# AnarchistHoneybun/map-oxidize

Measured on AMD Instinct MI355X. Metric: word-count input GB/s end-to-end at 1 and 8 MI355X; % of HBM peak, higher is better.
Workload: dtype u8

## Files before the change

map-oxidize_amd/csrc/mox_engine.hip:

```cpp
#include <fcntl.h>
#include <sys/stat.h>
#include <unistd.h>

#include <memory>

#include "mox_host.h"
#include "mox_unicode_tables.h"

namespace mox_host {

thread_local std::string g_err;

int fail(int code, const char* fmt, ...) {
  char buf[512];
  va_list ap;
  va_start(ap, fmt);
  vsnprintf(buf, sizeof buf, fmt, ap);
  va_end(ap);
  g_err = buf;
  return code;
}


int dalloc(mox_engine* e, void** p, size_t bytes) {
// ... 190 lines not shown
  memset(e->h_ctl_init, 0, sizeof(Ctl));
  e->h_ctl_init->err_utf8 = ~0ull;
  e->h_ctl_init->halo_err = ~0ull;
  return MOX_OK;
}

constexpr size_t map_lds_bytes() { return MAP_LDS_BYTES; }
size_t reduce_lds_bytes() { return RED_LDS_BYTES; }

float ev_ms(mox_engine* e, int a, int b) {
  float ms = 0;
  if (hipEventElapsedTime(&ms, e->ev[a], e->ev[b]) != hipSuccess) return 0;
  return ms;
}

void Seq::rec(int i) const {
  if ((i == 1 || i == 2) && map_ev[0]) {
    if (timing || map_only) (void)hipEventRecord(map_ev[i - 1], s);
    return;
  }
  if (timing || (map_only && (i == 1 || i == 2))) (void)hipEventRecord(e->ev[i], s);
}
void Seq::step(const char* name) const {
  if (!sync_each) return;
  hipError_t er = hipStreamSynchronize(s);
  fprintf(stderr, "[mox] %s done: %s\n", name, hipGetErrorString(er));
}

Seq seq_of(mox_engine* e) {
  const bool full = (e->flags & MOX_F_TIMING) != 0;
  return Seq{e, e->stream, full, e->sync_each, !full && (e->flags & MOX_F_TIMING_MAP) != 0};
}

void launch_reduce_tail(mox_engine* e, const Corpus& c, const Seq& q, bool zero) {
  Work& w = e->w;
  hipStream_t s = e->stream;
  hipLaunchKernelGGL(k_hist, dim3(w.map_grid), dim3(1024), 0, s, w);
  q.step("k_hist");
  hipLaunchKernelGGL(k_scatter, dim3(w.map_grid), dim3(1024), 0, s, w);
  q.step("k_scatter");
  hipLaunchKernelGGL(k_split_count, dim3(NB), dim3(256), 0, s, w);
  q.step("k_split_count");
  hipLaunchKernelGGL(k_unit_scan, dim3(1), dim3(256), 0, s, w);
  q.step("k_unit_scan");
  hipLaunchKernelGGL(k_split_scatter, dim3(NB), dim3(1024), 0, s, w);
  q.step("k_split_scatter");
  hipLaunchKernelGGL(k_reduce_sort1, dim3(MOX_S1_WG * e->n_cu), dim3(256), 0, s, w);
  q.step("k_reduce_sort1");
  hipLaunchKernelGGL(k_reduce_sort2, dim3(8 * e->n_cu), dim3(64), 0, s, w);
  q.step("k_reduce_sort2");
  hipLaunchKernelGGL(zero ? k_reduce_z : k_reduce, dim3(NB), dim3(RED_THREADS), reduce_lds_bytes(), s, w);
  q.step("k_reduce");
  hipLaunchKernelGGL(k_reduce_small, dim3(8 * e->n_cu), dim3(128), 0, s, w);
  q.step("k_reduce_small");
  q.rec(4);
  hipLaunchKernelGGL(k_unit_uniq_scan, dim3(NB), dim3(1024), 0, s, w);
  q.step("k_unit_uniq_scan");
  hipLaunchKernelGGL(k_final_scan, dim3(1), dim3(NB), 0, s, w);
  q.step("k_final_scan");
  hipLaunchKernelGGL(k_mat, dim3(std::max(NB, 6 * e->n_cu)), dim3(256), 0, s, w, c);
  q.step("k_mat");
  q.rec(5);
}

int finish_pass(mox_engine* e, const Seq& q) {
  HIPCHK(hipGetLastError());
  HIPCHK(hipMemcpyAsync(e->h_ctl, e->w.ctl, sizeof(Ctl), hipMemcpyDeviceToHost, e->stream));
  HIPCHK(hipStreamSynchronize(e->stream));
  if (q.map_only && !q.sync_each) {
    e->stats.ms_dict = e->stats.ms_lanes = e->stats.ms_reduce = e->stats.ms_finalize = e->stats.ms_run = 0;
    e->stats.ms_map = ev_ms(e, 1, 2);
  }
  if (q.timing) {
    e->stats.ms_dict = ev_ms(e, 0, 1);
    e->stats.ms_map = ev_ms(e, 1, 2);
    e->stats.ms_lanes = ev_ms(e, 2, 3);
    e->stats.ms_reduce = ev_ms(e, 3, 4);
    e->stats.ms_finalize = ev_ms(e, 4, 5);
    e->stats.ms_run = ev_ms(e, 0, 5);
  }
  return MOX_OK;
}

void launch_dict(mox_engine* e, const Corpus& c, hipStream_t s, const Seq& q) {
  Work& w = e->w;
  hipLaunchKernelGGL(k_sample, dim3(e->sample_pieces), dim3(256), 0, s, c, w, e->sample_pieces);
  q.step("k_sample");
  hipLaunchKernelGGL(k_dict_hist, dim3(GC_SLOTS / 1024), dim3(1024), 0, s, w);
  q.step("k_dict_hist");
  hipLaunchKernelGGL(k_dict_pick, dim3(GC_SLOTS / 1024), dim3(1024), 0, s, w, e->dict_words);
  q.step("k_dict_pick");
  hipLaunchKernelGGL(k_dict_build, dim3(1), dim3(1024), 0, s, w, e->dict_words);
  q.step("k_dict_build");
}

void enqueue_pass(mox_engine* e, const Corpus& c, const Seq& q, bool side = false) {
  Work& w = e->w;
  hipStream_t s = e->stream;
  q.rec(0);
  const bool dict = !(e->flags & MOX_F_NO_DICT) && c.own_hi > c.own_lo;
  const bool sided = side && dict && !q.timing && !q.sync_each;
  if (sided) {
    use_dset(e, e->dcur ^ 1);
    if (e->mapped_pending) (void)hipStreamWaitEvent(e->dstream, e->ev_mapped, 0);
    e->mapped_pending = false;
    hipLaunchKernelGGL(k_dict_zero, dim3(64), dim3(256), 0, e->dstream, w);
    launch_dict(e, c, e->dstream, q);
    (void)hipEventRecord(e->ev_dready, e->dstream);
  }
  hipLaunchKernelGGL(k_init, dim3(256), dim3(256), 0, s, w, 0ull, sided ? 4u : (dict ? 1u : 0u));
  q.step("k_init");
  if (sided) (void)hipStreamWaitEvent(s, e->ev_dready, 0);
  else if (dict) launch_dict(e, c, s, q);
  q.rec(1);
  const uint64_t row0 = c.own_lo & ~15ull;
  const uint64_t nrows = c.own_hi > c.own_lo ? (c.own_hi - row0 + PAY - 1) / PAY : 0;
  const int grid = (int)w.map_grid;
  hipLaunchKernelGGL(k_map, dim3(grid), dim3(MAP_THREADS), map_lds_bytes(), s, c, w, nrows, 0u);
  q.step("k_map");
  q.rec(2);
#ifndef MOX_SIDE_AFTER_MAP
#define MOX_SIDE_AFTER_MAP 0
#endif
  if (MOX_SIDE_AFTER_MAP && side && !q.timing && !q.sync_each) {
    (void)hipEventRecord(e->ev_mapped, s);
    e->mapped_pending = true;
  }
  hipLaunchKernelGGL(k_unicode, dim3(1024), dim3(256), 0, s, c, w, e->tables);
  q.step("k_unicode");
  q.rec(3);
  launch_reduce_tail(e, c, q, false);
}

int pipeline_once(mox_engine* e, const Corpus& c) {
  const Seq q = seq_of(e);
  enqueue_pass(e, c, q);
  return finish_pass(e, q);
}

uint64_t cold_cap_for(const mox_engine* e, const Ctl& h) {
  const uint64_t want = h.cold_need + h.cold_need / 8 + 16;
  const uint64_t bound = 4 * h.tokens / ((uint64_t)e->w.map_grid * NB) + 64;
  return std::min(want, std::max<uint64_t>(bound, e->w.cold_cap));
}

Caps grow_for(mox_engine* e, const Ctl& h) {
  Caps need = caps_of(e->w);
  if (h.overflow & OVF_POOL) {
    need.cold_cap = std::max<uint64_t>(need.cold_cap, cold_cap_for(e, h));
    need.spill_cap = std::max<uint64_t>(need.spill_cap, h.spill_need + h.spill_need / 4 + 1024);
  }
  if (h.overflow & OVF_W) {
    const uint64_t wn = std::max<uint64_t>(h.w_total, h.w_n);
    need.w_cap = std::max<uint64_t>(need.w_cap, wn + wn / 4 + 1024);
  }
  if (h.overflow & OVF_U) need.u_cap = h.u_n + h.u_n / 4 + 1024;
  if (h.overflow & OVF_ARENA) need.arena_cap = h.arena_n + h.arena_n / 4 + 65536;
  if (h.overflow & OVF_LONG) need.long_cap = next_pow2(2 * h.long_n + 1024);
  if (h.overflow & OVF_TABLE) need.table_cap = h.n_total + h.n_total / 4 + 1024;
  if (h.overflow & OVF_BYTES) need.bytes_cap = h.bytes_total + h.bytes_total / 4 + 65536;
  if (h.overflow & OVF_SPLIT) {
    uint64_t k = h.split_k + h.split_k / 8 + 4096, wv = h.split_w + h.split_w / 8 + 4096;
    if (need.split_k_cap || need.split_w_cap) {
      k = std::max<uint64_t>(k, h.cold_recs + h.cold_recs / 8 + (uint64_t)NB * (SUB_N + 2));
      wv = std::max<uint64_t>(wv, h.w_total + h.w_total / 8 + 4096);
    }
    need.split_k_cap = std::max<uint64_t>(need.split_k_cap, k);
    need.split_w_cap = std::max<uint64_t>(need.split_w_cap, wv);
  }
  if (h.overflow & OVF_TABLE) need.bytes_cap = std::max(need.bytes_cap, need.table_cap * 16);
  return need;
}

void commit_result(mox_engine* e, const Corpus& c, const Ctl& h);

void set_result(mox_engine* e, const Ctl& h) {
  e->res.counts = e->w.t_counts;
  e->res.offs = e->w.t_offs;
  e->res.bytes = e->w.t_bytes;
  e->res.n = h.n_total;
  e->res.nb = h.bytes_total;
  e->res.tokens = h.tokens;
  e->res.pass = true;
  e->res.exchanged = false;
  e->res.sorted = false;
  e->res.ranked = false;
  e->res.folded = false;
  e->have_result = true;
}
// ... 129 lines not shown
  if (&h != e->h_ctl) std::memcpy(e->h_ctl, &h, sizeof(Ctl));
  if (h.spill_need) e->next_cold_cap = std::max<uint64_t>(e->next_cold_cap, cold_cap_for(e, h));
  e->stats.bytes = c.own_hi - c.own_lo;
  e->stats.tokens = h.tokens;
  e->stats.uniques = h.n_total;
  e->stats.dict_words = h.dict_n;
  e->stats.cold_records = h.cold_recs;
  e->stats.weighted_records = h.w_n;
  e->stats.unicode_tokens = h.u_n;
  e->stats.long_tokens = h.long_n;
  e->stats.chunks = h.cold_need;
  e->stats.max_subpasses = h.max_sub ? h.max_sub : 1;
  e->stats.reduce_units = h.n_units;
  e->stats.split_partitions = h.n_split;
  static_assert(sizeof(e->stats.path_hits) == sizeof(h.paths), "path counters");
  std::memcpy(e->stats.path_hits, h.paths, sizeof h.paths);
  e->last_corpus = c;
  set_result(e, h);
}

int complete_async(mox_engine* e, int k) {
  auto& a = e->aslot[k];
  if (!a.pending) return MOX_OK;
  a.pending = false;
  HIPCHK(hipEventSynchronize(a.ev_done));
  const Ctl& h = *a.h_ctl;
  auto& later = e->aslot[k ^ 1];
  if (int rc = check_failed(h)) return rc;
  if (h.err_utf8 != ~0ull) return fail(MOX_EUTF8, "stream did not contain valid UTF-8 (byte %llu)", h.err_utf8);
  if (h.halo_err != ~0ull)
    return fail(MOX_EHALO, "token at byte %llu runs past the end of a non-final shard buffer", h.halo_err);
  if (!h.overflow) {
    const bool map_only = (e->flags & (MOX_F_TIMING | MOX_F_TIMING_MAP)) != 0;
    if (map_only) {
      float ms = 0;
      if (hipEventElapsedTime(&ms, a.ev_map0, a.ev_map1) == hipSuccess) e->stats.ms_map = ms;
    }
    e->stats.retries = 0;
    commit_result(e, a.c, h);
    if (later.pending) e->have_result = false;
    return MOX_OK;
  }
  if (later.pending) {
    e->grow_hint = caps_max(e->grow_hint, grow_for(e, h));
    e->stats.async_dropped++;
    return MOX_OK;
  }
  HIPCHK(hipStreamSynchronize(e->stream));
  if (e->dstream) HIPCHK(hipStreamSynchronize(e->dstream));
  e->stats.async_reruns++;
  return run_corpus(e, a.c);
}

int drain_async(mox_engine* e) {
  const int first = e->anext;
  int rc = complete_async(e, first);
  const int rc2 = complete_async(e, first ^ 1);
  if (e->dstream) HIPCHK(hipStreamSynchronize(e->dstream));
  return rc ? rc : rc2;
}

Corpus make_corpus(const void* d_buf, size_t buf_len, size_t own_begin, size_t own_end, int at_end) {
  uintptr_t addr = (uintptr_t)d_buf;
  uint64_t mis = (addr & 15) + 16;
  Corpus c{};
  c.base = (const uint8_t*)(addr - mis);
  c.lo = mis;
  c.hi = mis + buf_len;
  c.own_lo = mis + own_begin;
  c.own_hi = mis + own_end;
  c.ctx_lo = mis;
  c.at_end = at_end ? 1 : 0;
  return c;
}


int engine_create_one(const mox_config* cfg, int dev, mox_engine** out) {
  *out = nullptr;
  mox_engine* e = new (std::nothrow) mox_engine();
  if (!e) return fail(MOX_ENOMEM, "host allocation failed");
  if (cfg) {
    e->flags = cfg->flags;
    if (cfg->dict_words) e->dict_words = std::min<uint32_t>(cfg->dict_words, DICT_MAX_WORDS);
    if (cfg->sample_pieces) e->sample_pieces = std::min<uint32_t>(cfg->sample_pieces, MAX_SAMPLE_PIECES);
  }
  int ndev = 0;
  if (hipGetDeviceCount(&ndev) != hipSuccess || ndev == 0) {
    delete e;
    return fail(MOX_EHIP, "no HIP device available");
  }
  if (dev < 0) {
    if (hipGetDevice(&dev) != hipSuccess) dev = 0;
  }
  if (dev >= ndev) {
    delete e;
    return fail(MOX_EINVAL, "device %d out of range (%d devices)", dev, ndev);
  }
  e->device = dev;
  hipError_t herr = hipSetDevice(dev);
  if (herr != hipSuccess) { delete e; return fail(MOX_EHIP, "hipSetDevice: %s", hipGetErrorString(herr)); }
  hipDeviceProp_t prop;
  if (hipGetDeviceProperties(&prop, dev) == hipSuccess) e->n_cu = prop.multiProcessorCount;
  if (hipStreamCreateWithFlags(&e->stream, hipStreamNonBlocking) != hipSuccess) {
    delete e;
    return fail(MOX_EHIP, "hipStreamCreate failed");
  }
  for (auto& ev : e->ev) (void)hipEventCreate(&ev);
  if (hipStreamCreateWithFlags(&e->dstream, hipStreamNonBlocking) != hipSuccess ||
      hipEventCreateWithFlags(&e->ev_dready, hipEventDisableTiming) != hipSuccess ||
      hipEventCreateWithFlags(&e->ev_mapped, hipEventDisableTiming) != hipSuccess) {
    mox_engine_destroy(e);
    return fail(MOX_EHIP, "side stream / events: creation failed");
  }
  if (hipFuncSetAttribute((const void*)k_map, hipFuncAttributeMaxDynamicSharedMemorySize, (int)map_lds_bytes()) != hipSuccess ||
      hipFuncSetAttribute((const void*)k_reduce, hipFuncAttributeMaxDynamicSharedMemorySize, (int)reduce_lds_bytes()) != hipSuccess ||
      hipFuncSetAttribute((const void*)k_reduce_z, hipFuncAttributeMaxDynamicSharedMemorySize, (int)reduce_lds_bytes()) != hipSuccess) {
    mox_engine_destroy(e);
    return fail(MOX_EHIP, "hipFuncSetAttribute(dynamic LDS) failed");
  }
  if (const char* d = getenv("MOX_DBG")) e->w.dbg = (uint32_t)strtoul(d, nullptr, 0);
  if (e->w.dbg & DBG_STAMP) (void)hipMalloc((void**)&e->w.stamps, 8 * 8 * 4096 + 8 * 8 * 1024 * MAP_WAVES + 8 * 4 * 1024 * 16);
  e->sync_each = getenv("MOX_SYNC_EACH") != nullptr;
  e->verbose = getenv("MOX_VERBOSE") != nullptr;
  if (const char* f = getenv("MOX_TEST_FAIL_ALLOC")) e->test_fail_alloc = atoi(f);
  int rc = alloc_fixed(e);
  if (rc == MOX_OK && cfg && cfg->reserve_bytes) rc = ensure_caps(e, initial_caps(cfg->reserve_bytes, e->n_cu));
  if (rc != MOX_OK) {
    std::string msg = g_err;
    mox_engine_destroy(e);
    g_err = msg;
    return rc;
  }
  *out = e;
  return MOX_OK;
}

int stage_host_range(mox_engine* e, const uint8_t* text, size_t len) {
  if (len > e->d_text_cap) {
    dfree(e->d_text);
    e->d_text = nullptr;
    e->d_text_cap = 0;
    int rc = dalloc(e, (void**)&e->d_text, len + 64);
    if (rc) return rc;
    e->d_text_cap = len;
  }
  const bool timing = (e->flags & MOX_F_TIMING) != 0;
  if (timing) HIPCHK(hipEventRecord(e->ev[8], e->stream));
  if (len) HIPCHK(hipMemcpyAsync(e->d_text, text, len, hipMemcpyHostToDevice, e->stream));
  if (timing) HIPCHK(hipEventRecord(e->ev[9], e->stream));
  HIPCHK(hipStreamSynchronize(e->stream));
  if (timing) e->stats.ms_h2d = ev_ms(e, 8, 9);
  return MOX_OK;
}


constexpr int MAX_FILE_READERS = 16;
int file_readers() {
  static const int n = [] {
    const char* v = getenv("MOX_FILE_READERS");
    const int k = v ? atoi(v) : 8;
    return k < 1 ? 1 : (k > MAX_FILE_READERS ? MAX_FILE_READERS : k);
  }();
  return n;
}
bool file_shared_stream() {
  static const bool one = [] {
    const char* v = getenv("MOX_FILE_STREAMS");
// ... 626 lines not shown
```

map-oxidize_amd/csrc/mox_host.h:

```cpp
#pragma once
#include <fcntl.h>
#include <sys/mman.h>
#include <sys/stat.h>
#include <unistd.h>

#include <algorithm>
#include <atomic>
#include <condition_variable>
#include <chrono>
#include <cstdarg>
#include <cstdio>
#include <cstdlib>
#include <cstring>
#include <initializer_list>
#include <mutex>
#include <string>
#include <thread>
#include <vector>

#include <rccl/rccl.h>

#include "../../include/mox.h"
#include "mox_internal.h"
#include "mox_table.h"
// ... 10 lines not shown
__global__ void k_dict_build(Work w, uint32_t max_words);
__global__ void k_dict_zero(Work w);
__global__ void k_unicode(Corpus c, Work w, Tables T);
__global__ void k_hist(Work w);
__global__ void k_scatter(Work w);
__global__ void k_reduce(Work w);
__global__ void k_reduce_z(Work w);
__global__ void k_split_count(Work w);
__global__ void k_unit_scan(Work w);
__global__ void k_split_scatter(Work w);
__global__ void k_unit_uniq_scan(Work w);
__global__ void k_final_scan(Work w);
__global__ void k_reduce_small(Work w);
__global__ void k_reduce_sort1(Work w);
__global__ void k_reduce_sort2(Work w);
__global__ void k_mat(Work w, Corpus c);
__global__ void k_xcount(Work w, uint32_t P, XCnt* xcnt);
__global__ void k_xpack_short(Work w, WRec* out);
__global__ void k_xpack_long(Work w, XDir dir, unsigned long long* cur, uint8_t* blob);
__global__ void k_xsample(Work w, uint64_t* out);
__global__ void k_xsplit(const uint64_t* blocks, uint32_t P, uint64_t* sp, uint32_t* flag);
__global__ void k_xcount_r(Work w, XSplit x, XCnt* xcnt);
__global__ void k_xpack_r(Work w, XSplit x, XDir dir, unsigned long long* cur, WRec* out, uint8_t* blob);
__global__ void k_xingest(Work w, XDir dir, uint64_t n_short);
__global__ void k_gather_offs(const uint8_t* recv, GDir d, uint64_t* out);
}

namespace mox_host {
constexpr int GROW_RETRIES = 8;


extern thread_local std::string g_err;
int fail(int code, const char* fmt, ...) __attribute__((format(printf, 2, 3)));

#define HIPCHK(expr)                                                                             \
  do {                                                                                           \
    hipError_t e_ = (expr);                                                                      \
    if (e_ != hipSuccess) return fail(MOX_EHIP, "%s failed: %s (%s:%d)", #expr, hipGetErrorString(e_), __FILE__, __LINE__); \
  } while (0)

#define RCCLCHK(expr)                                                                            \
  do {                                                                                           \
    ncclResult_t r_ = (expr);                                                                    \
    if (r_ != ncclSuccess) return fail(MOX_ERCCL, "%s failed: %s", #expr, ncclGetErrorString(r_)); \
  } while (0)

inline uint64_t next_pow2(uint64_t x) {
  uint64_t p = 1;
  while (p < x) p <<= 1;
  return p;
}

struct DevBuf {
  void* p = nullptr;
  size_t cap = 0;
};
struct Caps {
  uint64_t cold_cap, spill_cap, w_cap, u_cap, arena_cap, long_cap, table_cap, bytes_cap, split_k_cap, split_w_cap;
};
struct XPlan;
struct Group;

}

using namespace mox_host;

struct mox_engine {
  int device = 0;
  hipStream_t stream = nullptr;
  hipStream_t dstream = nullptr;
  hipEvent_t ev_dready = nullptr;
  hipEvent_t ev_mapped = nullptr;
  bool mapped_pending = false;
  struct DictSet {
    WRec* cand = nullptr;
    uint32_t* dict_hist = nullptr;
    WRec* dict_list = nullptr;
    uint32_t* dict_tag = nullptr;
    uint4* dict_key = nullptr;
    unsigned long long* dict_tot = nullptr;
  } dsets[2];
  int dcur = 0;
  uint32_t flags = 0, dict_words = DICT_MAX_WORDS, sample_pieces = 192;
  int n_cu = 256;
  bool sync_each = false;
  bool verbose = false;
  int test_fail_alloc = 0;
  uint64_t next_cold_cap = 0;
  Caps grow_hint{};
  Work w{};
  Tables tables{};
  Ctl* h_ctl = nullptr;
  Ctl* h_ctl_init = nullptr;
  uint64_t* h_tot = nullptr;
  uint8_t* d_text = nullptr;
  size_t d_text_cap = 0;
  hipStream_t file_stream[16]{};
  hipEvent_t file_ev[16][2]{};
  hipEvent_t file_land = nullptr;
  uint8_t* file_pin[16][2]{};
  size_t file_pin_bytes = 0;
  bool have_result = false;
  struct Res {
    const uint64_t* counts = nullptr;
    const uint64_t* offs = nullptr;
    const uint8_t* bytes = nullptr;
    uint64_t n = 0, nb = 0, tokens = 0;
    bool pass = false;
    bool exchanged = false;
    bool sorted = false;
    bool ranked = false;
    bool folded = false;
  } res;
  struct Acc {
    bool have = false, sorted = false, ranked = false;
    uint64_t n = 0, nb = 0, tokens = 0, passes = 0;
  } acc;
  DevBuf a_tab[3], a_tc;
  DevBuf g_counts, g_offs, g_bytes, g_recv;
  DevBuf s_counts, s_offs, s_bytes, s_tmp;
  unsigned long long* h_bsort = nullptr;
  DevBuf k_tmp, k_out;
  DevBuf tx_pre, tx_slice[2], tx_pin[2];
  hipEvent_t tx_ev[2]{};
  DevBuf l_tmp, l_pin;
  DevBuf f_tab[2][3], f_tmp;
  DevBuf r_tab[2][3], r_tmp;
  uint64_t* h_rmax = nullptr;
  DevBuf q_tc;
  Corpus last_corpus{};
  mox_stats stats{};
  hipEvent_t ev[12]{};
  struct AsyncSlot {
    bool pending = false;
    Corpus c{};
    Ctl* h_ctl = nullptr;
    hipEvent_t ev_map0 = nullptr, ev_map1 = nullptr, ev_done = nullptr;
  } aslot[2];
  int anext = 0;
  ncclComm_t comm = nullptr;
  int nranks = 1, rank = 0;
  XCnt* d_xcnt = nullptr;
  XCnt* h_xcnt = nullptr;
  unsigned long long* d_xcur = nullptr;
  uint64_t* d_xs = nullptr;
  uint64_t* d_xr = nullptr;
  uint64_t* d_xsp = nullptr;
  uint32_t* h_xflag = nullptr;
  hipEvent_t ev_xs = nullptr;
  DevBuf x_send_short, x_send_blob, x_recv_short, x_recv_blob;
  DevBuf hx_send, hx_recv;
  Ctl* h_ctl_x = nullptr;
  XPlan* xp = nullptr;
  Group* grp = nullptr;
};

namespace mox_host {
int dalloc(mox_engine* e, void** p, size_t bytes);
void dfree(void* p);
Caps caps_of(const Work& w);
Caps initial_caps(uint64_t n, int map_grid);
Caps caps_max(const Caps& a, const Caps& b);
int ensure_caps(mox_engine* e, const Caps& need);
Caps grow_for(mox_engine* e, const Ctl& h);
int check_failed(const Ctl& h);
void set_result(mox_engine* e, const Ctl& h);
// ... 61 lines not shown
```

map-oxidize_amd/csrc/mox_internal.h:

```cpp
#pragma once
#include <hip/hip_runtime.h>
#include <stdint.h>

namespace mox {

constexpr int MAP_THREADS = 1024;
constexpr int MAP_WG_PER_CU = 1;
constexpr int MAP_MIN_WAVES = 1;
#if defined(MOX_ABLATE) && !defined(MOX_EXPERIMENT_BUILD)
#error "MOX_ABLATE is an experiment build (tools/build_variant.sh): not for the product library"
#endif
constexpr int MAP_LOADERS = 1;
#ifndef MOX_LD_SLEEP
#define MOX_LD_SLEEP 1
#endif
#ifndef MOX_CO_SLEEP
#define MOX_CO_SLEEP 1
#endif
#ifndef MOX_RING
#define MOX_RING 32
#endif
constexpr int RING = MOX_RING;
#ifndef MOX_DICT_SLOTS
#define MOX_DICT_SLOTS 5120
#endif
constexpr int DICT_SLOTS = MOX_DICT_SLOTS;
constexpr int DICT_MAX_WORDS = DICT_SLOTS < 4096 ? DICT_SLOTS : 4096;
constexpr size_t DICT_CNT_BYTES = (size_t)DICT_SLOTS * 4;
static_assert(DICT_SLOTS % 32 == 0 && DICT_SLOTS <= 65536 && DICT_MAX_WORDS <= DICT_SLOTS, "dictionary geometry");
constexpr int MAX_MAP_GRID = 1024;
constexpr int MAP_WAVES = MAP_THREADS / 64;
constexpr int ROW = 1024;
constexpr int ROWBUF = ROW + 32;
constexpr int TOKMAX = ROW / 2;
constexpr int SLOT = ROW;
constexpr int PAY = ROW - 32;
constexpr int KSEL_N = 17 * 4;
#ifndef MOX_LD_GROUPS
#define MOX_LD_GROUPS 4
#endif
#ifndef MOX_LD_GROUP
#define MOX_LD_GROUP 6
#endif
constexpr int LD_GROUP = MOX_LD_GROUP;
constexpr int LD_GROUPS = MOX_LD_GROUPS;
constexpr int MAP_CONSUMERS = MAP_WAVES - MAP_LOADERS;
constexpr int MAP_ROW_WAVES = MAP_CONSUMERS;
static_assert(TOKMAX - 1 >= PAY / 2, "list[TOKMAX - 1] is the token-loop sink: no row may reach it");
constexpr int LIST_N = TOKMAX + 64;
constexpr int NB_LOG2 = 10;
constexpr int NB = 1 << NB_LOG2;
constexpr uint64_t COLD_CAP_MAX = (1ull << 32) / (16ull * NB);
constexpr uint32_t QF_MAX = 4;
constexpr size_t MAP_LDS_BYTES = (size_t)DICT_SLOTS * 16 + DICT_CNT_BYTES + NB * 4 + 16 + KSEL_N * 16 +
                                 (size_t)RING * 8 + (size_t)RING * SLOT + (size_t)MAP_ROW_WAVES * 2 * LIST_N;
static_assert(MAP_LDS_BYTES <= 160 * 1024, "k_map LDS over 160 KiB");
constexpr int GC_SLOTS = 65536;
constexpr int MAX_SAMPLE_PIECES = 1024;
constexpr int SAMPLE_PIECE = 4096;
constexpr int SAMPLE_SLOTS = 2048;
constexpr int DH_N = 258, DH_T = 259;
constexpr int RED_THREADS = 1024;
constexpr int RED_BK = 608;
constexpr int RED_BUCKETS = RED_BK + 1;
constexpr int RED_SLOTS = 4 * RED_BUCKETS;
constexpr int RED_CAP = 2048;
constexpr int RED_SORTB = 2048;
constexpr size_t RED_LDS_BYTES = (size_t)RED_SLOTS * (4 + 16 + 8) + RED_CAP * 2 + (RED_SORTB + 8) * 2 + RED_SORTB * 2 + 16;
static_assert(RED_SLOTS * 4 % 16 == 0 && RED_LDS_BYTES + 256 <= 80 * 1024, "k_reduce LDS: 2 workgroups per CU");
constexpr int SUB_BITS_MAX = 12;
constexpr int SUB_N = 1 << SUB_BITS_MAX;
constexpr int U_MAX = NB * SUB_N;
constexpr int SUB_PER_T = SUB_N / 1024;
#ifndef MOX_SPLIT_MIN
#define MOX_SPLIT_MIN 8192
#endif
constexpr uint32_t SPLIT_MIN = MOX_SPLIT_MIN;
constexpr uint32_t SPLIT_TARGET = 320;
constexpr uint32_t SMALL_CAP = 512;
#ifndef MOX_S1_WG
#define MOX_S1_WG 4
#endif
#ifndef MOX_SPLIT_PER_REGION
#define MOX_SPLIT_PER_REGION 4
#endif
constexpr uint32_t SPLIT_PER_REGION = MOX_SPLIT_PER_REGION;
constexpr uint32_t SPLIT_SAMPLE = 256 * SPLIT_PER_REGION;
constexpr int LC_BITS = 4096;

constexpr uint64_t LONG_TAG = 0xFF00000000000000ull;
constexpr uint64_t LONG_LEN_MASK = 0x0000FFFFFFFFFFFFull;
constexpr uint64_t ARENA_BIT = 1ull << 63;

#ifdef MOX_ABLATE
#define MOX_ABL(d, f) (((d) & (f)) != 0)
#else
#define MOX_ABL(d, f) (false)
#endif
enum : uint32_t { DBG_NO_TOKENS = 1u, DBG_NO_EMIT = 2u, DBG_NO_DICT = 4u, DBG_NO_COLDSTORE = 8u, DBG_NO_DICTADD = 16u,
                  DBG_RED_NOSORT = 32u, DBG_RED_NOINSERT = 64u, DBG_RED_NOSLOW = 128u, DBG_COUNT = 256u, DBG_RED_PLAINADD = 512u, DBG_STAMP = 1024u,
                  DBG_RED_TWICE = 2048u,
                  DBG_NO_ROW = 4096u,
                  DBG_PAIR_NOSTORE = 8192u,
                  DBG_NOPAIR = 16384u,
                  DBG_PAIR_SEQ = 32768u,
                  DBG_S1_SORT2 = 65536u };
enum : uint32_t {
  CHK_SMALL_DESC = 1u, CHK_SMALL_OUT = 2u, CHK_RED_OUT = 3u, CHK_SPLIT_K = 4u, CHK_SPLIT_W = 5u, CHK_UNIT = 6u,
  CHK_MAT_ROW = 7u, CHK_MAT_BYTES = 8u, CHK_SCATTER = 9u, CHK_RED_IN = 10u, CHK_GATHER = 11u,
  CHK_RED_TABLE = 12u,
  CHK_RED_NU = 13u
};
#ifdef MOX_CHECK
#define MOX_CHK(w, ok, site) (::mox::chk_record((w).ctl, (ok), (site)))
#else
#define MOX_CHK(w, ok, site) (true)
#endif
enum : uint32_t {
  OVF_POOL = 1u, OVF_W = 2u, OVF_U = 4u, OVF_LONG = 8u, OVF_ARENA = 16u, OVF_PROBE = 32u,
  OVF_TABLE = 64u, OVF_BYTES = 128u, OVF_REDUCE = 256u, OVF_SPLIT = 512u,
  OVF_RERUN = OVF_POOL | OVF_W | OVF_U | OVF_LONG | OVF_ARENA | OVF_PROBE | OVF_SPLIT
};

struct Ctl {
  unsigned long long w_n;
  unsigned long long u_n;
  unsigned long long arena_n;
  unsigned long long long_n;
  unsigned long long long_uniq;
  unsigned long long tokens;
  unsigned long long err_utf8;
  unsigned long long halo_err;
  unsigned long long cold_recs;
  unsigned long long n_short;
  unsigned long long n_total;
  unsigned long long bytes_total;
  unsigned int overflow;
  unsigned int dict_n;
  unsigned int dict_maxprobe;
  unsigned int max_sub;
  unsigned int dict_thresh;
  unsigned int done[3];
  unsigned long long cold_need;
// ... 236 lines not shown
```

map-oxidize_amd/csrc/mox_kernels.hip:

```cpp
#include "mox_internal.h"

namespace mox {

__device__ __forceinline__ uint32_t movemask8(uint64_t m80) {
  uint64_t m = (m80 >> 7) & 0x0101010101010101ull;
  m |= m >> 7;
  m |= m >> 14;
  m |= m >> 28;
  return (uint32_t)m & 0xFFu;
}
__device__ __forceinline__ uint64_t zero_bytes80(uint64_t v) {
  uint64_t t = (v & 0x7F7F7F7F7F7F7F7Full) + 0x7F7F7F7F7F7F7F7Full;
  return ~(t | v | 0x7F7F7F7F7F7F7F7Full);
}
__device__ __forceinline__ uint64_t ws_bytes80(uint64_t x) {
  uint64_t sp = zero_bytes80(x ^ 0x2020202020202020ull);
  uint64_t ge9 = x + 0x7777777777777777ull;
  uint64_t ge14 = x + 0x7272727272727272ull;
  return (sp | (ge9 & ~ge14)) & 0x8080808080808080ull;
}
__device__ __forceinline__ uint64_t lower_ascii(uint64_t x) {
  uint64_t ge_a = x + 0x3F3F3F3F3F3F3F3Full;
  uint64_t gt_z = x + 0x2525252525252525ull;
  return x | (((ge_a & ~gt_z) & 0x8080808080808080ull) >> 2);
// ... 991 lines not shown
    for (uint32_t j = cnt; j < SPLIT_PER_REGION; j++) note_sample(m, b, q, j, 0u);
    cmax = cnt > cmax ? cnt : cmax;
  }
  for (int off = 32; off > 0; off >>= 1) {
    ntok += __shfl_down(ntok, off);
    const uint32_t o = __shfl_down(cmax, off);
    cmax = o > cmax ? o : cmax;
  }
  if (lane == 0) {
    if (ntok) atomicAdd(&s_tok, ntok);
    if (cmax) atomicMax(&s_cmax, cmax);
  }
  __syncthreads();
  if (tid == 0) {
    const uint32_t sn = m.s.misc[0];
    w.spill_n[blockIdx.x] = sn < w.spill_cap ? sn : w.spill_cap;
    if (sn) atomicMax(&w.ctl->spill_need, sn);
    if (s_cmax) atomicMax(&w.ctl->cold_need, (unsigned long long)s_cmax * m.qf);
    if (s_tok) atomicAdd(&w.ctl->tokens, s_tok);
    if (blockIdx.x == 0) w.ctl->qf = m.qf;
  }
}

extern "C" __global__ void k_ctl_out(const Ctl* __restrict__ src, Ctl* __restrict__ dst) {
  constexpr int CW = sizeof(Ctl) / 8;
  const int t = threadIdx.x;
  if (t < CW) reinterpret_cast<volatile unsigned long long*>(dst)[t] = reinterpret_cast<const unsigned long long*>(src)[t];
}

enum : uint32_t { INIT_DICT = 1u, INIT_MAP = 2u, INIT_DICT_SIDE = 4u };
__device__ __forceinline__ void zero_words(void* p, uint64_t bytes, uint64_t t, uint64_t stride) {
  uint4* q = reinterpret_cast<uint4*>(p);
  const uint64_t n16 = bytes / 16;
  for (uint64_t i = t; i < n16; i += stride) q[i] = make_uint4(0, 0, 0, 0);
  uint32_t* r = reinterpret_cast<uint32_t*>(q + n16);
  for (uint64_t i = t; i < (bytes % 16) / 4; i += stride) r[i] = 0;
}
extern "C" __global__ void k_init(Work w, unsigned long long w_n, uint32_t flags) {
  const uint64_t t = (uint64_t)blockIdx.x * blockDim.x + threadIdx.x, stride = (uint64_t)gridDim.x * blockDim.x;
  constexpr int CW = sizeof(Ctl) / 8;
  static_assert(sizeof(Ctl) % 8 == 0, "Ctl is zeroed in 8-byte words");
  if (t < CW) {
    unsigned long long* c = reinterpret_cast<unsigned long long*>(w.ctl);
    const uint64_t off = t * 8;
    unsigned long long v = 0;
    if (off == offsetof(Ctl, err_utf8) || off == offsetof(Ctl, halo_err)) v = ~0ull;
    if (off == offsetof(Ctl, w_n)) v = w_n;
    c[t] = v;
  }
  zero_words(w.b_recs, NB * 8, t, stride);
  zero_words(w.b_w, NB * 4, t, stride);
  zero_words(w.ltab, w.long_cap * sizeof(LSlot), t, stride);
  if (flags & INIT_DICT) {
    zero_words(w.cand, (uint64_t)GC_SLOTS * sizeof(WRec), t, stride);
    zero_words(w.dict_hist, 260 * 4, t, stride);
  }
  if (flags & (INIT_DICT | INIT_DICT_SIDE)) zero_words(w.dict_tot, DICT_SLOTS * 8, t, stride);
  else if (t == 0) { w.dict_hist[DH_N] = 0; w.dict_hist[DH_T] = 0; }
  if (flags & INIT_MAP) {
    zero_words(w.cold_n, (uint64_t)w.map_grid * NB * QF_MAX * 4, t, stride);
    zero_words(w.samp, (uint64_t)w.map_grid * NB * QF_MAX * SPLIT_PER_REGION * 4, t, stride);
    zero_words(w.spill_n, (uint64_t)w.map_grid * 4, t, stride);
  }
}

extern "C" __global__ void k_dict_zero(Work w) {
  const uint64_t t = (uint64_t)blockIdx.x * blockDim.x + threadIdx.x, stride = (uint64_t)gridDim.x * blockDim.x;
  zero_words(w.cand, (uint64_t)GC_SLOTS * sizeof(WRec), t, stride);
  zero_words(w.dict_hist, 260 * 4, t, stride);
}
__device__ __forceinline__ bool claim16(unsigned long long* k0, unsigned long long* k1, uint64_t w0, uint64_t w1) {
  const unsigned long long t1 = w1 | (1ull << 63);
  unsigned long long o0 = atomicCAS(k0, 0ull, (unsigned long long)w0);
  if (o0 != 0 && o0 != w0) return false;
  unsigned long long o1 = atomicCAS(k1, 0ull, t1);
  return o1 == 0 || o1 == t1;
}

__device__ __forceinline__ uint32_t lower32(uint32_t x) {
  const uint32_t ge_a = x + 0x3F3F3F3Fu, gt_z = x + 0x25252525u;
  return x | (((ge_a & ~gt_z) & 0x80808080u) >> 2);
}

extern "C" __global__ __launch_bounds__(256) void k_sample(Corpus c, Work w, uint32_t npieces) {
  constexpr int BUF = SAMPLE_PIECE + 48;
  __shared__ __attribute__((aligned(16))) uint8_t buf[BUF];
  __shared__ unsigned long long sk0[SAMPLE_SLOTS], sk1[SAMPLE_SLOTS];
  __shared__ uint32_t scnt[SAMPLE_SLOTS];
  __shared__ uint4 mtab[17];
  const int tid = threadIdx.x;
  for (int i = tid; i < SAMPLE_SLOTS; i += 256) { sk0[i] = 0; sk1[i] = 0; scnt[i] = 0; }
  if (tid < 17) {
    uint32_t mk[4];
#pragma unroll
    for (int i = 0; i < 4; i++) {
      const int cc = tid - 4 * i;
      mk[i] = cc <= 0 ? 0u : (cc >= 4 ? ~0u : ((1u << (8 * cc)) - 1u));
    }
    mtab[tid] = make_uint4(mk[0], mk[1], mk[2], mk[3]);
  }
  const uint64_t span = c.own_hi - c.own_lo;
  const uint64_t stride = span / npieces;
  const uint64_t ps = (c.own_lo + stride * blockIdx.x) & ~15ull;
  for (int i = tid; i < BUF / 16; i += 256) {
    const uint64_t p = ps - 16 + (uint64_t)i * 16;
    const bool in = p + 16 > c.lo && p < c.hi;
    reinterpret_cast<uint4*>(buf)[i] = in ? fix16(c, p, raw16(c, p)) : make_uint4(0x20202020u, 0x20202020u, 0x20202020u, 0x20202020u);
  }
  __syncthreads();
  const uint4 own = reinterpret_cast<const uint4*>(buf)[1 + tid], nxt = reinterpret_cast<const uint4*>(buf)[2 + tid];
  const uint32_t prevb = buf[15 + 16 * tid];
  const uint32_t ws32 = ws_mask16(own) | (ws_mask16(nxt) << 16);
  uint32_t start = (~ws32) & ((ws32 << 1) | (is_ascii_ws(prevb) ? 1u : 0u)) & 0xFFFFu;
  while (start) {
    const uint32_t p = __builtin_ctz(start);
    start &= start - 1;
    const uint32_t rest = ws32 >> p;
    const uint32_t len = rest ? __builtin_ctz(rest) : 32;
    if (len > 16) continue;
    const uint32_t pos = 16 + 16 * tid + p;
    const uint2* q = reinterpret_cast<const uint2*>(buf + (pos & ~7u));
    const uint2 A = q[0], B = q[1], C = q[2];
    const uint4 M = mtab[len];
    const bool o = (pos & 4u) != 0;
    const uint32_t E0 = o ? A.y : A.x, E1 = o ? B.x : A.y, E2 = o ? B.y : B.x, E3 = o ? C.x : B.y, E4 = o ? C.y : C.x;
    const uint32_t sh = pos & 3u;
    uint32_t K[4] = {__builtin_amdgcn_alignbyte(E1, E0, sh) & M.x, __builtin_amdgcn_alignbyte(E2, E1, sh) & M.y,
                     __builtin_amdgcn_alignbyte(E3, E2, sh) & M.z, __builtin_amdgcn_alignbyte(E4, E3, sh) & M.w};
    if (((K[0] | K[1] | K[2] | K[3]) & 0x80808080u) != 0) continue;
    const uint32_t nz = (uint32_t)__popcll(zero_bytes80(((uint64_t)K[1] << 32) | K[0])) +
                        (uint32_t)__popcll(zero_bytes80(((uint64_t)K[3] << 32) | K[2]));
    if (nz != 16 - len) continue;
#pragma unroll
    for (int i = 0; i < 4; i++) K[i] = lower32(K[i]);
    const uint64_t w0 = ((uint64_t)K[1] << 32) | K[0], w1 = ((uint64_t)K[3] << 32) | K[2];
    uint32_t slot = hash32(K[0], K[1], K[2], K[3]) & (SAMPLE_SLOTS - 1);
    for (int pr = 0; pr < 64; pr++) {
      if (claim16(&sk0[slot], &sk1[slot], w0, w1)) { atomicAdd(&scnt[slot], 1u); break; }
      slot = (slot + 1) & (SAMPLE_SLOTS - 1);
    }
  }
  __syncthreads();
  __shared__ uint16_t lw[SAMPLE_SLOTS];
  __shared__ uint32_t nlw;
  if (tid == 0) nlw = 0;
  __syncthreads();
  for (int i = tid; i < SAMPLE_SLOTS; i += 256) {
    const bool used = scnt[i] != 0 && sk0[i] != 0 && sk1[i] != 0;
    const uint64_t bm = __ballot(used);
    uint32_t b0 = 0;
    if ((tid & 63) == 0 && bm) b0 = atomicAdd(&nlw, (uint32_t)__popcll(bm));
    b0 = __shfl(b0, 0);
    if (used) lw[b0 + (uint32_t)__popcll(bm & ((1ull << (tid & 63)) - 1ull))] = (uint16_t)i;
  }
  __syncthreads();
  for (uint32_t j = tid; j < nlw; j += 256) {
    const uint32_t i = lw[j];
    const uint32_t n = scnt[i];
    const uint64_t w0 = sk0[i], w1 = sk1[i] & ~(1ull << 63);
    uint32_t g = key_hash(w0, w1) & (GC_SLOTS - 1);
    for (int pr = 0; pr < 16; pr++) {
      WRec* r = &w.cand[g];
      if (claim16((unsigned long long*)&r->w0, (unsigned long long*)&r->w1, w0, w1)) {
        atomicAdd((unsigned long long*)&r->count, (unsigned long long)n);
        break;
      }
      g = (g + 1) & (GC_SLOTS - 1);
    }
  }
}

extern "C" __global__ __launch_bounds__(1024) void k_dict_hist(Work w) {
  __shared__ uint32_t h[256];
  if (threadIdx.x < 256) h[threadIdx.x] = 0;
  __syncthreads();
  for (uint32_t i = blockIdx.x * 1024 + threadIdx.x; i < GC_SLOTS; i += gridDim.x * 1024) {
    const uint64_t n = w.cand[i].count;
    if (n) atomicAdd(&h[n > 255 ? 255 : n], 1u);
  }
  __syncthreads();
  if (threadIdx.x < 256 && h[threadIdx.x]) atomicAdd(&w.dict_hist[threadIdx.x], h[threadIdx.x]);
}

constexpr uint32_t DICT_MIN_COVER_INV = 20;
extern "C" __global__ __launch_bounds__(1024) void k_dict_pick(Work w, uint32_t max_words) {
  __shared__ uint32_t T, ST, h[256];
  __shared__ unsigned long long cov[2];
  if (threadIdx.x < 256) h[threadIdx.x] = w.dict_hist[threadIdx.x];
  __syncthreads();
  {
    __shared__ uint64_t wsum[16];
    uint64_t tot;
    const int cc = 255 - (int)threadIdx.x;
    const uint64_t x = threadIdx.x < 256 ? h[cc] : 0;
    const uint64_t ex = block_exscan(x, wsum, tot);
    if (threadIdx.x == 0) { T = 256; ST = 0; }
    __syncthreads();
    if (threadIdx.x < 254 && ex + x <= max_words) atomicMin(&T, (uint32_t)cc);
    __syncthreads();
    if (threadIdx.x < 256 && cc == (int)T) ST = (uint32_t)(ex + x);
    if (threadIdx.x == 0) {
      if (T > 255) T = 256;
      cov[0] = 0;
      cov[1] = 0;
    }
    __syncthreads();
    if (threadIdx.x < 256 && cc >= 1 && x) {
      const unsigned long long tok = x * (unsigned long long)cc;
      atomicAdd(&cov[0], tok);
      if ((uint32_t)cc >= T) atomicAdd(&cov[1], tok);
    }
    __syncthreads();
    if (threadIdx.x == 0) {
      if (cov[1] < cov[0] / DICT_MIN_COVER_INV) T = 256;
      if (blockIdx.x == 0) w.dict_hist[DH_T] = T;
    }
    __syncthreads();
  }
  __shared__ uint32_t wn[2][16], base[2];
  const uint32_t t = T, t1 = T - 1;
  const uint32_t i = blockIdx.x * 1024 + threadIdx.x;
  const WRec r = w.cand[i];
  const bool real = r.w0 != 0 && r.w1 != 0;
  const bool pick = real && r.count >= t;
  const bool fill = real && t1 >= 2 && t1 < 255 && r.count == t1;
  const uint64_t bm = __ballot(pick), bf = __ballot(fill);
  const int lane = threadIdx.x & 63, wv = threadIdx.x >> 6;
  if (lane == 0) { wn[0][wv] = (uint32_t)__popcll(bm); wn[1][wv] = (uint32_t)__popcll(bf); }
  __syncthreads();
  const uint64_t lt = (1ull << lane) - 1ull;
  uint32_t pre = (uint32_t)__popcll(bm & lt), pref = (uint32_t)__popcll(bf & lt), tot = 0, totf = 0;
  for (int k = 0; k < 16; k++) {
    if (k < wv) { pre += wn[0][k]; pref += wn[1][k]; }
    tot += wn[0][k];
    totf += wn[1][k];
  }
  if (threadIdx.x == 0) {
    base[0] = tot ? atomicAdd(&w.dict_hist[256], tot) : 0u;
    base[1] = totf ? atomicAdd(&w.dict_hist[257], totf) : 0u;
  }
  __syncthreads();
  if (pick) {
    const uint32_t o = base[0] + pre;
    if (o < max_words) w.dict_list[o] = WRec{r.w0, r.w1 & ~(1ull << 63), r.count};
  } else if (fill) {
    const uint32_t o = ST + base[1] + pref;
    if (o < max_words) w.dict_list[o] = WRec{r.w0, r.w1 & ~(1ull << 63), r.count};
  }
}

extern "C" __global__ __launch_bounds__(1024) void k_dict_build(Work w, uint32_t max_words) {
  __shared__ uint32_t ltag[DICT_SLOTS];
  __shared__ uint16_t lword[DICT_SLOTS];
  __shared__ uint32_t klock[DICT_SLOTS / 32];
  __shared__ uint2 lk0[DICT_MAX_WORDS], lk1[DICT_MAX_WORDS];
  __shared__ uint8_t lcl[DICT_MAX_WORDS];
  __shared__ uint16_t order[DICT_MAX_WORDS];
  __shared__ uint16_t fails[DICT_MAX_WORDS];
  __shared__ uint32_t ccnt[32], cstart[33], cfill[32];
  __shared__ uint32_t nsel, nfail;
  const int tid = threadIdx.x;
  for (int i = tid; i < DICT_SLOTS; i += 1024) ltag[i] = 0;
  for (int i = tid; i < DICT_SLOTS / 32; i += 1024) klock[i] = 0;
  if (tid < 32) { ccnt[tid] = 0; cfill[tid] = 0; }
  if (tid == 0) nsel = 0;
  uint32_t n = w.dict_hist[256] + w.dict_hist[257];
  if (n > max_words) n = max_words;
  __syncthreads();
  for (uint32_t i = tid; i < n; i += 1024) {
    const WRec r = w.dict_list[i];
    const uint32_t cnt = r.count > 0xFFFFFFFFull ? 0xFFFFFFFFu : (uint32_t)r.count;
    lk0[i] = make_uint2((uint32_t)r.w0, (uint32_t)(r.w0 >> 32));
    lk1[i] = make_uint2((uint32_t)r.w1, (uint32_t)(r.w1 >> 32));
    lcl[i] = (uint8_t)(31 - __clz(cnt | 1u));
    atomicAdd(&ccnt[lcl[i]], 1u);
  }
  __syncthreads();
  if (tid == 0) {
    uint32_t a = 0;
    for (int cl = 31; cl >= 0; cl--) { cstart[cl] = a; a += ccnt[cl]; }
    cstart[32] = a;
  }
  __syncthreads();
  for (uint32_t i = tid; i < n; i += 1024) order[cstart[lcl[i]] + atomicAdd(&cfill[lcl[i]], 1u)] = (uint16_t)i;
  __syncthreads();
  for (int cl = 31; cl >= 0; cl--) {
    const uint32_t c0 = cstart[cl], c1 = c0 + ccnt[cl];
    if (c0 == c1) continue;
    if (tid == 0) nfail = 0;
    __syncthreads();
    for (uint32_t j = c0 + tid; j < c1; j += 1024) {
      const uint32_t i = order[j];
      const uint2 a = lk0[i], b = lk1[i];
      const uint32_t h = hash32(a.x, a.y, b.x, b.y);
      int slot = -1;
      if (atomicCAS(&ltag[dict_s1(h)], 0u, h) == 0u) slot = (int)dict_s1(h);
      else if (atomicCAS(&ltag[dict_s2(h)], 0u, h) == 0u) slot = (int)dict_s2(h);
      if (slot < 0) { fails[atomicAdd(&nfail, 1u)] = (uint16_t)i; continue; }
      lword[slot] = (uint16_t)i;
    }
    __syncthreads();
    const uint32_t nf = nfail;
    for (uint32_t j = tid; j < nf; j += 1024) {
      const uint32_t i = fails[j];
      const uint2 a = lk0[i], b = lk1[i];
      const uint32_t h = hash32(a.x, a.y, b.x, b.y);
      const uint32_t xs[2] = {dict_s1(h), dict_s2(h)};
      for (int q = 0; q < 2; q++) {
        const uint32_t x = xs[q];
        if (atomicOr(&klock[x >> 5], 1u << (x & 31)) & (1u << (x & 31))) continue;
        const uint32_t ho = ltag[x];
        const uint32_t alt = dict_s1(ho) == x ? dict_s2(ho) : dict_s1(ho);
        if (alt == x) continue;
        if (atomicOr(&klock[alt >> 5], 1u << (alt & 31)) & (1u << (alt & 31))) continue;
// ... 1913 lines not shown
```

Baseline: 993.9.

## Shrink k_sample LDS so it co-resides with k_map and scale sample count

Rewrites k_sample to keep a small 32-bit hash-tag table in LDS (about 4 KiB) instead of a 4 KiB text buffer plus full 16-byte keys. Tokens are re-derived from registers and emitted in a second pass by their first occurrence, with overflow words going straight to the global candidate table. This lets sample workgroups fit beside the persistent k_map on the side stream. It also grows the sample count with input size up to a larger default and doubles GC_SLOTS. The cost is hash-tag collisions merging distinct words into one count, more global atomics on overflow, and more sampling work.

```diff
diff --git a/map-oxidize_amd/csrc/mox_engine.hip b/map-oxidize_amd/csrc/mox_engine.hip
--- a/map-oxidize_amd/csrc/mox_engine.hip
+++ b/map-oxidize_amd/csrc/mox_engine.hip
@@ -296,9 +296,16 @@
   return MOX_OK;
 }
 
+uint32_t sample_count(const mox_engine* e, const Corpus& c, bool side) {
+  if (!side) return e->sample_pieces;
+  const uint64_t fit = (c.own_hi - c.own_lo) / (SAMPLE_PIECE + 16);
+  return (uint32_t)std::min<uint64_t>(e->sample_pieces_max, std::max<uint64_t>(e->sample_pieces, fit));
+}
+
 void launch_dict(mox_engine* e, const Corpus& c, hipStream_t s, const Seq& q) {
   Work& w = e->w;
-  hipLaunchKernelGGL(k_sample, dim3(e->sample_pieces), dim3(256), 0, s, c, w, e->sample_pieces);
+  const uint32_t pieces = sample_count(e, c, s == e->dstream);
+  hipLaunchKernelGGL(k_sample, dim3(pieces), dim3(256), 0, s, c, w, pieces);
   q.step("k_sample");
   hipLaunchKernelGGL(k_dict_hist, dim3(GC_SLOTS / 1024), dim3(1024), 0, s, w);
   q.step("k_dict_hist");
@@ -318,7 +325,7 @@
     use_dset(e, e->dcur ^ 1);
     if (e->mapped_pending) (void)hipStreamWaitEvent(e->dstream, e->ev_mapped, 0);
     e->mapped_pending = false;
-    hipLaunchKernelGGL(k_dict_zero, dim3(64), dim3(256), 0, e->dstream, w);
+    hipLaunchKernelGGL(k_dict_zero, dim3(128), dim3(256), 0, e->dstream, w);
     launch_dict(e, c, e->dstream, q);
     (void)hipEventRecord(e->ev_dready, e->dstream);
   }
@@ -614,7 +621,7 @@
   if (cfg) {
     e->flags = cfg->flags;
     if (cfg->dict_words) e->dict_words = std::min<uint32_t>(cfg->dict_words, DICT_MAX_WORDS);
-    if (cfg->sample_pieces) e->sample_pieces = std::min<uint32_t>(cfg->sample_pieces, MAX_SAMPLE_PIECES);
+    if (cfg->sample_pieces) e->sample_pieces = e->sample_pieces_max = std::min<uint32_t>(cfg->sample_pieces, MAX_SAMPLE_PIECES);
   }
   int ndev = 0;
   if (hipGetDeviceCount(&ndev) != hipSuccess || ndev == 0) {
diff --git a/map-oxidize_amd/csrc/mox_host.h b/map-oxidize_amd/csrc/mox_host.h
--- a/map-oxidize_amd/csrc/mox_host.h
+++ b/map-oxidize_amd/csrc/mox_host.h
@@ -116,6 +116,7 @@
   } dsets[2];
   int dcur = 0;
   uint32_t flags = 0, dict_words = DICT_MAX_WORDS, sample_pieces = 192;
+  uint32_t sample_pieces_max = DEFAULT_SAMPLE_PIECES;
   int n_cu = 256;
   bool sync_each = false;
   bool verbose = false;
diff --git a/map-oxidize_amd/csrc/mox_internal.h b/map-oxidize_amd/csrc/mox_internal.h
--- a/map-oxidize_amd/csrc/mox_internal.h
+++ b/map-oxidize_amd/csrc/mox_internal.h
@@ -55,10 +55,13 @@
 constexpr size_t MAP_LDS_BYTES = (size_t)DICT_SLOTS * 16 + DICT_CNT_BYTES + NB * 4 + 16 + KSEL_N * 16 +
                                  (size_t)RING * 8 + (size_t)RING * SLOT + (size_t)MAP_ROW_WAVES * 2 * LIST_N;
 static_assert(MAP_LDS_BYTES <= 160 * 1024, "k_map LDS over 160 KiB");
-constexpr int GC_SLOTS = 65536;
-constexpr int MAX_SAMPLE_PIECES = 1024;
+constexpr int GC_SLOTS = 131072;
+constexpr int MAX_SAMPLE_PIECES = 2048;
+constexpr int DEFAULT_SAMPLE_PIECES = 768;
 constexpr int SAMPLE_PIECE = 4096;
-constexpr int SAMPLE_SLOTS = 2048;
+constexpr int SAMPLE_SLOTS = 512;
+constexpr int SAMPLE_PROBES = 8;
+static_assert(MAP_LDS_BYTES + 1280 + 4096 <= 160 * 1024, "no room for a k_sample workgroup beside k_map (1,280 B LDS granule)");
 constexpr int DH_N = 258, DH_T = 259;
 constexpr int RED_THREADS = 1024;
 constexpr int RED_BK = 608;
diff --git a/map-oxidize_amd/csrc/mox_kernels.hip b/map-oxidize_amd/csrc/mox_kernels.hip
--- a/map-oxidize_amd/csrc/mox_kernels.hip
+++ b/map-oxidize_amd/csrc/mox_kernels.hip
@@ -1097,34 +1097,33 @@
   return x | (((ge_a & ~gt_z) & 0x80808080u) >> 2);
 }
 
-extern "C" __global__ __launch_bounds__(256) void k_sample(Corpus c, Work w, uint32_t npieces) {
-  constexpr int BUF = SAMPLE_PIECE + 48;
-  __shared__ __attribute__((aligned(16))) uint8_t buf[BUF];
-  __shared__ unsigned long long sk0[SAMPLE_SLOTS], sk1[SAMPLE_SLOTS];
-  __shared__ uint32_t scnt[SAMPLE_SLOTS];
-  __shared__ uint4 mtab[17];
-  const int tid = threadIdx.x;
-  for (int i = tid; i < SAMPLE_SLOTS; i += 256) { sk0[i] = 0; sk1[i] = 0; scnt[i] = 0; }
-  if (tid < 17) {
-    uint32_t mk[4];
-#pragma unroll
-    for (int i = 0; i < 4; i++) {
-      const int cc = tid - 4 * i;
-      mk[i] = cc <= 0 ? 0u : (cc >= 4 ? ~0u : ((1u << (8 * cc)) - 1u));
-    }
-    mtab[tid] = make_uint4(mk[0], mk[1], mk[2], mk[3]);
-  }
-  const uint64_t span = c.own_hi - c.own_lo;
-  const uint64_t stride = span / npieces;
-  const uint64_t ps = (c.own_lo + stride * blockIdx.x) & ~15ull;
-  for (int i = tid; i < BUF / 16; i += 256) {
-    const uint64_t p = ps - 16 + (uint64_t)i * 16;
-    const bool in = p + 16 > c.lo && p < c.hi;
-    reinterpret_cast<uint4*>(buf)[i] = in ? fix16(c, p, raw16(c, p)) : make_uint4(0x20202020u, 0x20202020u, 0x20202020u, 0x20202020u);
-  }
-  __syncthreads();
-  const uint4 own = reinterpret_cast<const uint4*>(buf)[1 + tid], nxt = reinterpret_cast<const uint4*>(buf)[2 + tid];
-  const uint32_t prevb = buf[15 + 16 * tid];
+__device__ __forceinline__ void cand_add(const Work& w, uint64_t w0, uint64_t w1, uint32_t n) {
+  uint32_t g = key_hash(w0, w1) & (GC_SLOTS - 1);
+  for (int pr = 0; pr < 16; pr++) {
+    WRec* r = &w.cand[g];
+    if (claim16((unsigned long long*)&r->w0, (unsigned long long*)&r->w1, w0, w1)) {
+      atomicAdd((unsigned long long*)&r->count, (unsigned long long)n);
+      return;
+    }
+    g = (g + 1) & (GC_SLOTS - 1);
+  }
+}
+__device__ __forceinline__ uint4 sample16(const Corpus& c, uint64_t p) {
+  const bool in = p + 16 > c.lo && p < c.hi;
+  return in ? fix16(c, p, raw16(c, p)) : make_uint4(0x20202020u, 0x20202020u, 0x20202020u, 0x20202020u);
+}
+
+__device__ __forceinline__ uint32_t sample_hash(const uint32_t* K) {
+  uint32_t h = K[0] * 0x9E3779B1u;
+  h = (h ^ K[1]) * 0x85EBCA77u;
+  h = (h ^ K[2]) * 0xC2B2AE3Du;
+  h = (h ^ K[3]) * 0x27D4EB2Fu;
+  h ^= h >> 15;
+  return h | 0x80000000u;
+}
+
+template <class F>
+__device__ __forceinline__ void sample_tokens(const uint4 own, const uint4 nxt, const uint32_t prevb, F&& f) {
   const uint32_t ws32 = ws_mask16(own) | (ws_mask16(nxt) << 16);
   uint32_t start = (~ws32) & ((ws32 << 1) | (is_ascii_ws(prevb) ? 1u : 0u)) & 0xFFFFu;
   while (start) {
@@ -1133,56 +1132,67 @@
     const uint32_t rest = ws32 >> p;
     const uint32_t len = rest ? __builtin_ctz(rest) : 32;
     if (len > 16) continue;
-    const uint32_t pos = 16 + 16 * tid + p;
-    const uint2* q = reinterpret_cast<const uint2*>(buf + (pos & ~7u));
-    const uint2 A = q[0], B = q[1], C = q[2];
-    const uint4 M = mtab[len];
-    const bool o = (pos & 4u) != 0;
-    const uint32_t E0 = o ? A.y : A.x, E1 = o ? B.x : A.y, E2 = o ? B.y : B.x, E3 = o ? C.x : B.y, E4 = o ? C.y : C.x;
-    const uint32_t sh = pos & 3u;
-    uint32_t K[4] = {__builtin_amdgcn_alignbyte(E1, E0, sh) & M.x, __builtin_amdgcn_alignbyte(E2, E1, sh) & M.y,
-                     __builtin_amdgcn_alignbyte(E3, E2, sh) & M.z, __builtin_amdgcn_alignbyte(E4, E3, sh) & M.w};
+    const uint32_t D[8] = {own.x, own.y, own.z, own.w, nxt.x, nxt.y, nxt.z, nxt.w};
+    const uint32_t j = p >> 2, sh = p & 3u;
+    uint32_t E[5];
+#pragma unroll
+    for (int k = 0; k < 5; k++) E[k] = j == 0 ? D[k] : (j == 1 ? D[k + 1] : (j == 2 ? D[k + 2] : D[k + 3]));
+    uint32_t K[4];
+#pragma unroll
+    for (int k = 0; k < 4; k++) {
+      const int cc = (int)len - 4 * k;
+      const uint32_t mk = cc <= 0 ? 0u : (cc >= 4 ? ~0u : ((1u << (8 * cc)) - 1u));
+      K[k] = __builtin_amdgcn_alignbyte(E[k + 1], E[k], sh) & mk;
+    }
     if (((K[0] | K[1] | K[2] | K[3]) & 0x80808080u) != 0) continue;
     const uint32_t nz = (uint32_t)__popcll(zero_bytes80(((uint64_t)K[1] << 32) | K[0])) +
                         (uint32_t)__popcll(zero_bytes80(((uint64_t)K[3] << 32) | K[2]));
     if (nz != 16 - len) continue;
 #pragma unroll
     for (int i = 0; i < 4; i++) K[i] = lower32(K[i]);
-    const uint64_t w0 = ((uint64_t)K[1] << 32) | K[0], w1 = ((uint64_t)K[3] << 32) | K[2];
-    uint32_t slot = hash32(K[0], K[1], K[2], K[3]) & (SAMPLE_SLOTS - 1);
-    for (int pr = 0; pr < 64; pr++) {
-      if (claim16(&sk0[slot], &sk1[slot], w0, w1)) { atomicAdd(&scnt[slot], 1u); break; }
+    f(p, K, sample_hash(K));
+  }
+}
+
+extern "C" __global__ __launch_bounds__(256) void k_sample(Corpus c, Work w, uint32_t npieces) {
+  __shared__ uint32_t stag[SAMPLE_SLOTS], scnt[SAMPLE_SLOTS];
+  static_assert(SAMPLE_SLOTS % 256 == 0 && SAMPLE_SLOTS * 8 <= 4096, "k_sample: LDS at most 4 KiB");
+  static_assert(SAMPLE_PIECE == 256 * 16 && SAMPLE_PIECE <= 1 << 12, "scnt: piece offset in the 12 bits above a 20-bit count");
+  const int tid = threadIdx.x;
+  for (int i = tid; i < SAMPLE_SLOTS; i += 256) { stag[i] = 0; scnt[i] = 0; }
+  const uint64_t span = c.own_hi - c.own_lo;
+  const uint64_t stride = span / npieces;
+  const uint64_t ps = (c.own_lo + stride * blockIdx.x) & ~15ull;
+  const uint64_t pt = ps + 16 * (uint64_t)tid;
+  const uint4 own = sample16(c, pt), nxt = sample16(c, pt + 16);
+  uint32_t prevw = __shfl_up(own.w, 1);
+  if ((tid & 63) == 0) prevw = sample16(c, pt - 16).w;
+  const uint32_t prevb = prevw >> 24;
+  __syncthreads();
+  sample_tokens(own, nxt, prevb, [&](uint32_t p, const uint32_t* K, uint32_t h) {
+    uint32_t slot = h & (SAMPLE_SLOTS - 1);
+    for (int pr = 0; pr < SAMPLE_PROBES; pr++) {
+      const uint32_t o = atomicCAS(&stag[slot], 0u, h);
+      if (o == 0u || o == h) {
+        atomicAdd(&scnt[slot], o == 0u ? (((uint32_t)tid * 16 + p) << 20) | 1u : 1u);
+        return;
+      }
       slot = (slot + 1) & (SAMPLE_SLOTS - 1);
     }
-  }
-  __syncthreads();
-  __shared__ uint16_t lw[SAMPLE_SLOTS];
-  __shared__ uint32_t nlw;
-  if (tid == 0) nlw = 0;
-  __syncthreads();
-  for (int i = tid; i < SAMPLE_SLOTS; i += 256) {
-    const bool used = scnt[i] != 0 && sk0[i] != 0 && sk1[i] != 0;
-    const uint64_t bm = __ballot(used);
-    uint32_t b0 = 0;
-    if ((tid & 63) == 0 && bm) b0 = atomicAdd(&nlw, (uint32_t)__popcll(bm));
-    b0 = __shfl(b0, 0);
-    if (used) lw[b0 + (uint32_t)__popcll(bm & ((1ull << (tid & 63)) - 1ull))] = (uint16_t)i;
-  }
-  __syncthreads();
-  for (uint32_t j = tid; j < nlw; j += 256) {
-    const uint32_t i = lw[j];
-    const uint32_t n = scnt[i];
-    const uint64_t w0 = sk0[i], w1 = sk1[i] & ~(1ull << 63);
-    uint32_t g = key_hash(w0, w1) & (GC_SLOTS - 1);
-    for (int pr = 0; pr < 16; pr++) {
-      WRec* r = &w.cand[g];
-      if (claim16((unsigned long long*)&r->w0, (unsigned long long*)&r->w1, w0, w1)) {
-        atomicAdd((unsigned long long*)&r->count, (unsigned long long)n);
-        break;
+    cand_add(w, ((uint64_t)K[1] << 32) | K[0], ((uint64_t)K[3] << 32) | K[2], 1u);
+  });
+  __syncthreads();
+  sample_tokens(own, nxt, prevb, [&](uint32_t p, const uint32_t* K, uint32_t h) {
+    uint32_t slot = h & (SAMPLE_SLOTS - 1);
+    for (int pr = 0; pr < SAMPLE_PROBES; pr++) {
+      if (stag[slot] == h) {
+        const uint32_t n = scnt[slot];
+        if (n >> 20 == (uint32_t)tid * 16 + p) cand_add(w, ((uint64_t)K[1] << 32) | K[0], ((uint64_t)K[3] << 32) | K[2], n & 0xFFFFFu);
+        return;
       }
-      g = (g + 1) & (GC_SLOTS - 1);
-    }
-  }
+      slot = (slot + 1) & (SAMPLE_SLOTS - 1);
+    }
+  });
 }
 
 extern "C" __global__ __launch_bounds__(1024) void k_dict_hist(Work w) {
@@ -1245,6 +1255,7 @@
   __syncthreads();
   const uint64_t lt = (1ull << lane) - 1ull;
   uint32_t pre = (uint32_t)__popcll(bm & lt), pref = (uint32_t)__popcll(bf & lt), tot = 0, totf = 0;
+#pragma unroll 1
   for (int k = 0; k < 16; k++) {
     if (k < wv) { pre += wn[0][k]; pref += wn[1][k]; }
     tot += wn[0][k];
```

Result: no change. 1002, median of 6 (+0.8%).
